# pvjosue/CWFA

Hardware: AMD Instinct MI355X
Metric: volumes/sec inverse-pass @512×512×96 fp32; NLL match vs ref (1/2/4/8 GPU) (higher is better)
Workload: dtype f32 (storage, accumulation, wavelets, couplings); convolution products on the bf16 matrix cores from an exact three-way bf16 split of both fp32 operands, six products per fp32 product: fp32-equivalent; plain-fp32-MFMA figure: fp32_mfma; 1 GPU; 512x512x96 volume, 4-scale CWFA (CAT blocks, 64 ch) + LRNN inverse, z=0, batch 1/GPU, random-init weights (BASELINE.json configs[2]); precision=split, parallelism=replicated x1 (independent volumes per GPU, no collective)

## Files before the change

### cwfa_amd/csrc/conv_split3x3.hip

```cpp
#include "conv_internal.h"

extern int g_cwfa_split_xcd_map;
extern int g_cwfa_split_rows16;

namespace {

constexpr int TR = 8, TC = 32;

template <int KS, int RPW = 4>
struct XG {
    static constexpr int TRW = 2 * RPW, NT = 2 * RPW;
    static constexpr int PAD = KS / 2, XR = TRW + 2 * PAD, XC = TC + 2 * PAD, NTAP = KS * KS;
    static constexpr int EPK = XR * XC;
    static constexpr int KHB = KS == 7 ? 8512 : RPW == 8 ? 9792 : 5440;
    static constexpr int XPB = 2 * KHB;
    static constexpr int XB = 3 * XPB;
    static constexpr bool SPECIAL = KS == 3 && RPW == 4;
    static constexpr int NEK = SPECIAL ? 2 : 3;
    static_assert(EPK * 16 <= KHB && KHB % 256 == 64 && 2 * EPK <= 512 * NEK, "staging entry map");
    static_assert(!SPECIAL || (EPK > 256 && EPK <= 384), "3x3 staging entry map");
    static_assert(KS == 3 || RPW == 4, "7x7: 8-row tiles");
};

template <int MPW, int KS = 3, int RPW = 4, int WM = 4>
struct Geo {
    static constexpr int CT = 16 * MPW * WM;
    static constexpr int WSL = 3 * 4 * CT * 16;
    static constexpr int LDS = 2 * XG<KS, RPW>::XB + 2 * WSL;
    static_assert(LDS <= 160 * 1024, "LDS budget");
};

struct SParams {
    const float* x;
    const void* wp;
    float* y;
    int B, Cin, H, W, Cout, nchunks, nsteps, tiles_x, ntiles, ctiles, xcd_map;
    int nrun;
    int64_t x_bs, y_bs;
    cwfa_conv_opts o;
    cwfa_couple cp;
};

template <int KS, int RPW>
__host__ __device__ constexpr int tap_off(int buf, int tap) { return buf * XG<KS, RPW>::XB + ((tap / KS) * XG<KS, RPW>::XC + tap % KS) * 16; }

enum { EPI_RUNTIME = -1, EPI_COUPLE = -2 };

template <int MPW, bool SIX, bool ADD, int ACT1, int KS = 3, int RPW = 4, int WM = 4, bool F16 = false>
__global__ __launch_bounds__(512, 1) void conv3x3_split_kernel(SParams p) {
    typedef XG<KS, RPW> G;
    constexpr int XC = G::XC, EPK = G::EPK, KHB = G::KHB, XPB = G::XPB, XB = G::XB, NTAP = G::NTAP, PAD = G::PAD;
    constexpr int WN = 8 / WM, RW = G::TRW / WN, NT = 2 * RW;
    constexpr bool SPECIAL = G::SPECIAL;
    static_assert(SPECIAL || ((MPW == 1 || WM != 4) && !ADD), "7x7 / 16-row tiles: the 64-channel and narrow tilings, without a skip add");
    static_assert(WM == 4 || (((KS == 3 && RPW == 8) || KS == 7) && MPW <= 3 && !ADD && ACT1 != EPI_COUPLE),
                  "narrow tilings: 16-row tile (7x7: 8-row), <= 3 m-tiles per wave");
    static_assert(MPW != 3 || WM != 4, "three m-tiles per wave: the 48- / 96-channel tilings only");
    constexpr int CT = 16 * MPW * WM;
    constexpr int WSL = 3 * 4 * CT * 16;
    extern __shared__ __attribute__((aligned(16))) char lds[];
    const int tid = threadIdx.x, lane = tid & 63, c16 = lane & 15, g = lane >> 4;
    const int wave = __builtin_amdgcn_readfirstlane(tid >> 6);
    const int wm = wave % WM, wn = wave / WM;
    const int HW = p.H * p.W;
    const int plane = HW * 4;
    constexpr unsigned OOB = 0x80000000u;
    constexpr int NQ = SIX ? 3 : 1;
    constexpr int OFF_W = 2 * XB;
    const int b = blockIdx.z;
    int sp, ct;
    if (p.xcd_map && (p.ntiles & 7) == 0) {
        const int xcd = blockIdx.x & 7, slot = blockIdx.x >> 3;
        sp = xcd * (p.ntiles >> 3) + slot / p.ctiles;
        ct = slot % p.ctiles;
    } else {
        sp = blockIdx.x / p.ctiles;
        ct = blockIdx.x % p.ctiles;
    }
    const int row0 = (sp / p.tiles_x) * G::TRW, col0 = (sp % p.tiles_x) * TC;

    constexpr int NEK = G::NEK;
    int ekh[NEK], eidx[NEK];
    bool fin[NEK];
    unsigned fo[NEK];
    if constexpr (SPECIAL) {
        ekh[0] = wave >> 2; eidx[0] = tid & 255; fin[0] = true;
        ekh[1] = (wave >> 1) & 1; eidx[1] = 256 + (tid & 127); fin[1] = wave < 4 && eidx[1] < EPK;
    } else {
#pragma unroll
        for (int k = 0; k < NEK; ++k) {
            const int e = tid + 512 * k;
            ekh[k] = e >= EPK;
            eidx[k] = e - ekh[k] * EPK;
            fin[k] = e < 2 * EPK;
        }
    }
    bool fok[NEK];
#pragma unroll
    for (int k = 0; k < NEK; ++k) {
        const int r = eidx[k] / XC, c = eidx[k] % XC;
        const int gr = row0 + r - PAD, gc = col0 + c - PAD;
        fok[k] = fin[k] && gr >= 0 && gr < p.H && gc >= 0 && gc < p.W;
        fo[k] = !fok[k] ? OOB : p.o.in_blocked8 ? (unsigned)((gr * p.W + gc) * 32) : (unsigned)((gr * p.W + gc) * 4);
        if constexpr (!SPECIAL) fo[k] = !fok[k] ? OOB : fo[k] + (unsigned)(ekh[k] * 8) * (unsigned)plane;
    }
    const int xbytes = p.Cin * plane;
    const auto rx = CWFA_RSRC(p.x + (int64_t)b * p.x_bs, xbytes);
    const auto ra = CWFA_RSRC(ADD ? p.o.in_add + (int64_t)b * p.o.in_add_bs : p.x, ADD ? xbytes : 0);
    const bool has_aff = p.o.in_scale != nullptr;
    typedef const float __attribute__((address_space(4))) cfloat;
    cfloat* sc = has_aff ? (cfloat*)(p.o.in_scale + (int64_t)b * p.o.in_affine_bs) : nullptr;
    cfloat* sh = has_aff ? (cfloat*)(p.o.in_shift + (int64_t)b * p.o.in_affine_bs) : nullptr;

    auto load_entry = [&](auto kc, float (&xv)[8], float (&av)[8], int chunk) {
        constexpr int k = decltype(kc)::value;
        const int ch0 = chunk * 16 + (SPECIAL ? ekh[k] * 8 : 0);
        if (KS == 3 && !ADD && p.o.in_blocked8) {
            const f32x4 lo4 = __builtin_bit_cast(f32x4, __builtin_amdgcn_raw_buffer_load_b128(rx, fo[k], ch0 * plane, 0));
            const f32x4 hi4 = __builtin_bit_cast(f32x4, __builtin_amdgcn_raw_buffer_load_b128(rx, fo[k], ch0 * plane + 16, 0));
#pragma unroll
            for (int j = 0; j < 4; ++j) {
                xv[j] = lo4[j];
                xv[4 + j] = hi4[j];
            }
            return;
        }
#pragma unroll
        for (int j = 0; j < 8; ++j) xv[j] = __builtin_bit_cast(float, __builtin_amdgcn_raw_buffer_load_b32(rx, fo[k], (ch0 + j) * plane, 0));
        if constexpr (ADD) {
#pragma unroll
            for (int j = 0; j < 8; ++j) av[j] = __builtin_bit_cast(float, __builtin_amdgcn_raw_buffer_load_b32(ra, fo[k], (ch0 + j) * plane, 0));
        }
    };
    auto store_entry = [&](auto kc, const float (&xv)[8], const float (&av)[8], int chunk, int buf) {
        constexpr int k = decltype(kc)::value;
        if (SPECIAL && k == 1 && !fin[1]) return;
        const int ch0 = chunk * 16 + ekh[k] * 8;
        bf16x8 pc[3];
        float scv[8], shv[8];
        if (has_aff) {
#pragma unroll
            for (int j = 0; j < 8; ++j) {
                const int ch = ch0 + j < p.Cin ? ch0 + j : p.Cin - 1;
                scv[j] = ch0 + j < p.Cin ? sc[ch] : 0.f;
                shv[j] = ch0 + j < p.Cin ? sh[ch] : 0.f;
            }
        }
#pragma unroll
        for (int j = 0; j < 8; ++j) {
            float v = xv[j];
            if (has_aff) v = fok[k] ? v * scv[j] + shv[j] : 0.f;
            if constexpr (ADD) v += av[j];
            __bf16 a1, a2 = (__bf16)0.f, a3 = (__bf16)0.f;
            cwfa_split3<SIX, F16>(v, a1, a2, a3);
            pc[0][j] = a1; pc[1][j] = a2; pc[2][j] = a3;
        }
        char* dst = lds + buf * XB + ekh[k] * KHB + eidx[k] * 16;
        if (SPECIAL || fin[k]) {
#pragma unroll
            for (int q = 0; q < NQ; ++q) *reinterpret_cast<bf16x8*>(dst + q * XPB) = pc[q];
        }
    };

    constexpr int NPC = (SIX ? WSL : WSL / 3) / 1024;
    const int64_t wtile = (int64_t)ct * p.nsteps * WSL;
    const char* wbase = reinterpret_cast<const char*>(p.wp) + wtile;
    const auto rw = CWFA_RSRC(wbase, p.nsteps * WSL);
    auto dma_w = [&](int slice, int slot) {
        cwfa_static_for<(NPC + 7) / 8>([&](auto ic_) {
            constexpr int i = decltype(ic_)::value;
            const int piece = i * 8 + wave;
            if (piece < NPC) {
                char* dst = lds + OFF_W + slot * WSL + piece * 1024;
                __builtin_amdgcn_raw_ptr_buffer_load_lds(rw, (lds_ptr)dst, 16, (unsigned)(lane * 16), slice * WSL + piece * 1024, 0, 0);
            }
        });
    };

    const int alane = OFF_W + (g * CT + wm * MPW * 16 + c16) * 16;
    const int blane = (g & 1) * KHB + (wn * RW * XC + c16) * 16;
    const bool sel = (g >> 1) != 0;

    f32x4 acc[MPW][NT];
#pragma unroll
    for (int mt = 0; mt < MPW; ++mt)
#pragma unroll
        for (int nt = 0; nt < NT; ++nt) acc[mt][nt] = f32x4{0.f, 0.f, 0.f, 0.f};
    constexpr int NB = MPW == 4 ? 3 : 2, MA = MPW == 4 ? 2 : MPW;
    static_assert(NB - 1 < NT, "B look-ahead");
    bf16x8 A[MPW][3], Bq[NB][3];
    float xs[NEK][8], sk[NEK][8];

    auto read_a = [&](int abase, int m0, int m1) {
#pragma unroll
        for (int mt = m0; mt < m1; ++mt)
#pragma unroll
            for (int q = 0; q < NQ; ++q) A[mt][q] = *reinterpret_cast<const bf16x8*>(lds + abase + (q * 4 * CT + mt * 16) * 16);
    };
    auto read_b = [&](int set, int bbase, int nt) {
#pragma unroll
        for (int q = 0; q < NQ; ++q)
            Bq[set][q] = *reinterpret_cast<const bf16x8*>(lds + bbase + q * XPB + ((nt >> 1) * XC + 16 * (nt & 1)) * 16);
    };
    auto mfma6 = [&](f32x4& c, const bf16x8 (&a)[3], const bf16x8 (&bb)[3]) {
        if constexpr (SIX) {
            CWFA_MFMA(a[2], bb[0], c);
            CWFA_MFMA(a[1], bb[1], c);
            CWFA_MFMA(a[0], bb[2], c);
            CWFA_MFMA(a[1], bb[0], c);
            CWFA_MFMA(a[0], bb[1], c);
        }
        CWFA_MFMA_OP(F16, a[0], bb[0], c);
    };

    {
        float x0[NEK][8], s0[NEK][8];
        cwfa_static_for<NEK>([&](auto kc) { load_entry(kc, x0[decltype(kc)::value], s0[decltype(kc)::value], 0); });
        cwfa_static_for<NEK>([&](auto kc) { load_entry(kc, xs[decltype(kc)::value], sk[decltype(kc)::value], 1); });
        dma_w(0, 0);
        cwfa_static_for<NEK>([&](auto kc) { store_entry(kc, x0[decltype(kc)::value], s0[decltype(kc)::value], 0, 0); });
    }
    asm volatile("s_waitcnt vmcnt(0)\n\ts_waitcnt lgkmcnt(0)" ::: "memory");
    __builtin_amdgcn_s_barrier();

    read_b(0, blane + (sel ? tap_off<KS, RPW>(0, 1) : tap_off<KS, RPW>(0, 0)), 0);
    int sl = 0, P = 0, ce = 0;
    for (int step = 0; step < p.nrun; ++step) {
        const int co = ce + 1;
        const int uA = 2 * P, uB = 2 * P + 1;
        const int bufA = uA >= NTAP, tA = uA - NTAP * bufA, bufB = uB >= NTAP, tB = uB - NTAP * bufB;
        const int offA = bufA * XB + ((tA / KS) * XC + tA % KS) * 16, offB = bufB * XB + ((tB / KS) * XC + tB % KS) * 16;
        constexpr int SB = 0, SA = KS == 3 ? 5 : 26, LA = KS == 3 ? 2 : 22, LB = KS == 3 ? 6 : 44;
        static_assert(LB + NEK - 1 < NTAP && LA + NEK - 1 < SA, "staging schedule");
        static_assert(SB < LA && SA <= LB, "staging schedule: one register set per entry (a step's stores come before its loads)");
        {
            const bool odd0 = P == SB, odd1 = P == SB + 1;
            if (odd0 || P == SA) store_entry(cwfa_ic<0>{}, xs[0], sk[0], odd0 ? co : ce + 2, odd0);
            if (odd1 || P == SA + 1) store_entry(cwfa_ic<1>{}, xs[1], sk[1], odd1 ? co : ce + 2, odd1);
            if constexpr (NEK > 2) {
                const bool odd2 = P == SB + 2;
                if (odd2 || P == SA + 2) store_entry(cwfa_ic<NEK - 1>{}, xs[NEK - 1], sk[NEK - 1], odd2 ? co : ce + 2, odd2);
            }
        }
        CWFA_FENCE();
        const int abase = alane + sl * WSL;
        const int bbase = blane + (sel ? offB : offA);
        read_a(abase, 0, MA);
        CWFA_FENCE();
#pragma unroll
        for (int nt = 0; nt < NT; ++nt) {
            if ((MA == MPW || nt > 0) && nt + NB - 1 < NT) read_b((nt + NB - 1) % NB, bbase, nt + NB - 1);
            CWFA_FENCE();
#pragma unroll
            for (int mt = 0; mt < MPW; ++mt) {
                mfma6(acc[mt][nt], A[mt], Bq[nt % NB]);
                CWFA_FENCE();
                if (MA < MPW && nt == 0 && mt == 0) {
                    read_a(abase, MA, MPW);
#pragma unroll
                    for (int n2 = 1; n2 < NB && n2 < NT; ++n2) read_b(n2, bbase, n2);
                    CWFA_FENCE();
                }
            }
            if (nt == 0) {
                if (P == LA || P == LB) load_entry(cwfa_ic<0>{}, xs[0], sk[0], P == LA ? ce + 2 : co + 2);
                if (P == LA + 1 || P == LB + 1) load_entry(cwfa_ic<1>{}, xs[1], sk[1], P == LA + 1 ? ce + 2 : co + 2);
                if constexpr (NEK > 2) {
                    if (P == LA + 2 || P == LB + 2) load_entry(cwfa_ic<NEK - 1>{}, xs[NEK - 1], sk[NEK - 1], P == LA + 2 ? ce + 2 : co + 2);
                }
                CWFA_FENCE();
            }
            if (nt == 1) {
                dma_w(step + 1, sl ^ 1);
                CWFA_FENCE();
            }
        }
        {
            const int nP = P == NTAP - 1 ? 0 : P + 1;
            const int nA = 2 * nP, nB = 2 * nP + 1;
            const int nbufA = nA >= NTAP, ntA = nA - NTAP * nbufA, nbufB = nB >= NTAP, ntB = nB - NTAP * nbufB;
            const int noffA = nbufA * XB + ((ntA / KS) * XC + ntA % KS) * 16, noffB = nbufB * XB + ((ntB / KS) * XC + ntB % KS) * 16;
            read_b(0, blane + (sel ? noffB : noffA), 0);
            CWFA_FENCE();
        }
        asm volatile("s_waitcnt vmcnt(0)" ::: "memory");
        if constexpr (SIX) asm volatile("s_waitcnt lgkmcnt(3)" ::: "memory");
        else asm volatile("s_waitcnt lgkmcnt(1)" ::: "memory");
        __builtin_amdgcn_s_barrier();
        sl ^= 1;
        if (++P == NTAP) {
            P = 0;
            ce += 2;
        }
    }
    asm volatile("s_waitcnt vmcnt(0)" ::: "memory");

    const auto ry = CWFA_RSRC(p.y + (int64_t)b * p.y_bs, p.Cout * plane);
    const auto rr = CWFA_RSRC(p.o.residual ? p.o.residual + (int64_t)b * p.o.res_bs : p.y, p.o.residual ? p.Cout * plane : 0);
    const auto rb = CWFA_RSRC(p.o.bias ? p.o.bias : p.y, p.o.bias ? p.Cout * 4 : 0);
    const bool alpha_pc = p.o.prelu_per_channel != 0;
    const float alpha = (p.o.prelu_alpha && !alpha_pc) ? *p.o.prelu_alpha : 0.f;
    const auto rpa = CWFA_RSRC(alpha_pc ? p.o.prelu_alpha : p.y, alpha_pc ? p.Cout * 4 : 0);
    const int cwave = ct * CT + wm * MPW * 16;
    const unsigned glane = (unsigned)(4 * g) * (unsigned)plane;
    if constexpr (ACT1 == EPI_COUPLE) {
        static_assert(MPW <= 2 && !ADD, "coupling epilogue: narrow tilings only");
        constexpr int NP = MPW == 1 ? 2 : 4;
        const cwfa_couple& cp = p.cp;
        const auto cx = CWFA_RSRC(cp.x + (int64_t)b * cp.x_bs, cp.n * plane);
        const auto cy = CWFA_RSRC(cp.y + (int64_t)b * cp.y_bs, cp.n * plane);
        const unsigned jlane = (unsigned)((MPW == 1 ? 2 : 4) * g) * (unsigned)plane;
        const int jwave = wm * (MPW == 1 ? 8 : 16);
        float bs[NP], bt[NP];
#pragma unroll
        for (int k = 0; k < NP; ++k) {
            const int rs = k, rt = MPW == 1 ? k + 2 : 16 + k;
            bs[k] = __builtin_bit_cast(float, __builtin_amdgcn_raw_buffer_load_b32(rb, (unsigned)(16 * g), (cwave + rs) * 4, 0));
            bt[k] = __builtin_bit_cast(float, __builtin_amdgcn_raw_buffer_load_b32(rb, (unsigned)(16 * g), (cwave + rt) * 4, 0));
        }
        float ssum = 0.f;
#pragma unroll
        for (int nt = 0; nt < NT; ++nt) {
            const int row = row0 + wn * RW + (nt >> 1), col = col0 + 16 * (nt & 1) + c16;
            const bool ok = row < p.H && col < p.W;
            const unsigned po = ok ? (unsigned)((row * p.W + col) * 4) + jlane : OOB;
            float xv[NP];
#pragma unroll
            for (int k = 0; k < NP; ++k) xv[k] = __builtin_bit_cast(float, __builtin_amdgcn_raw_buffer_load_b32(cx, po, (jwave + k) * plane, 0));
#pragma unroll
            for (int k = 0; k < NP; ++k) {
                const float sr = acc[0][nt][k] + bs[k];
                float tr;
                if constexpr (MPW == 1) tr = acc[0][nt][k + 2] + bt[k];
                else tr = acc[MPW - 1][nt][k] + bt[k];
                const float sv = cwfa_soft_clamp(sr * cp.pre_scale, cp.clamp_kind, cp.clamp);
                const float tv = tr * cp.pre_scale;
                const float yv = cp.rev ? (xv[k] - tv) * __expf(-sv) : __expf(sv) * xv[k] + tv;
                __builtin_amdgcn_raw_buffer_store_b32(__builtin_bit_cast(unsigned, yv), cy, po, (jwave + k) * plane, 0);
                ssum += ok ? sv : 0.f;
            }
            CWFA_FENCE();
        }
        if (cp.logdet) {
            const double ws = cwfa_wave_sum((double)ssum);
            double* red = reinterpret_cast<double*>(lds);
            __builtin_amdgcn_s_barrier();
            if (lane == 0) red[wave] = ws;
            __syncthreads();
            if (tid == 0) {
                double tot = 0.0;
#pragma unroll
                for (int w = 0; w < 8; ++w) tot += red[w];
                atomicAdd(&cp.logdet[b], cp.rev ? -tot : tot);
            }
        }
        return;
    }
    const bool outb = p.o.out_blocked8 != 0;
    const bool want_stats = ACT1 != EPI_RUNTIME && p.o.out_stats != nullptr;
    float* red = reinterpret_cast<float*>(lds);
#pragma unroll
    for (int mt = 0; mt < MPW; ++mt) {
        float bias[4];
        float st1[4] = {0.f, 0.f, 0.f, 0.f}, st2[4] = {0.f, 0.f, 0.f, 0.f};
#pragma unroll
        for (int r = 0; r < 4; ++r)
            bias[r] = __builtin_bit_cast(float, __builtin_amdgcn_raw_buffer_load_b32(rb, (unsigned)(16 * g), (cwave + mt * 16 + r) * 4, 0));
        float al[4] = {alpha, alpha, alpha, alpha};
        if (alpha_pc) {
#pragma unroll
            for (int r = 0; r < 4; ++r)
                al[r] = __builtin_bit_cast(float, __builtin_amdgcn_raw_buffer_load_b32(rpa, (unsigned)(16 * g), (cwave + mt * 16 + r) * 4, 0));
        }
        constexpr int RLA = NT < 4 ? NT : 4;
        float rv[ACT1 == EPI_RUNTIME ? NT : 1][4];
        auto load_res = [&](int nt) {
            const int row = row0 + wn * RW + (nt >> 1), col = col0 + 16 * (nt & 1) + c16;
            const unsigned po = (row < p.H && col < p.W) ? (unsigned)((row * p.W + col) * 4) + glane : OOB;
#pragma unroll
            for (int r = 0; r < 4; ++r)
                rv[ACT1 == EPI_RUNTIME ? nt : 0][r] = __builtin_bit_cast(float, __builtin_amdgcn_raw_buffer_load_b32(rr, po, (cwave + mt * 16 + r) * plane, 0));
        };
        if constexpr (ACT1 == EPI_RUNTIME) {
#pragma unroll
            for (int nt = 0; nt < NT; ++nt)
#pragma unroll
                for (int r = 0; r < 4; ++r) rv[nt][r] = 0.f;
            if (p.o.residual) {
#pragma unroll
                for (int nt = 0; nt < RLA; ++nt) load_res(nt);
            }
            CWFA_FENCE();
        }
#pragma unroll
        for (int nt = 0; nt < NT; ++nt) {
            const int row = row0 + wn * RW + (nt >> 1), col = col0 + 16 * (nt & 1) + c16;
            if constexpr (ACT1 == EPI_RUNTIME) {
                if (nt + RLA < NT && p.o.residual) load_res(nt + RLA);
                CWFA_FENCE();
            }
            if constexpr (ACT1 != EPI_RUNTIME) {
                if (outb) {
                    f32x4 o4;
#pragma unroll
                    for (int r = 0; r < 4; ++r) o4[r] = cwfa_act_ct<ACT1>(acc[mt][nt][r] + bias[r], al[r]);
                    const unsigned pb = (row < p.H && col < p.W) ? (unsigned)(((g >> 1) * HW + row * p.W + col) * 32 + (g & 1) * 16) : OOB;
                    cwfa_buffer_store_b128(__builtin_bit_cast(u32x4, o4), ry, pb, (cwave + mt * 16) * plane);
                    continue;
                }
            }
            const unsigned po = (row < p.H && col < p.W) ? (unsigned)((row * p.W + col) * 4) + glane : OOB;
#pragma unroll
            for (int r = 0; r < 4; ++r) {
                const int soff = (cwave + mt * 16 + r) * plane;
                float v = acc[mt][nt][r] + bias[r];
                if constexpr (ACT1 == EPI_RUNTIME) {
                    v = cwfa_act(v, p.o.act, al[r]);
                    v += rv[nt][r];
                    v = cwfa_act(v, p.o.act2, al[r]);
                } else {
                    v = cwfa_act_ct<ACT1>(v, al[r]);
                    if (want_stats) {
                        const float vm = po != OOB ? v : 0.f;
                        st1[r] += vm;
                        st2[r] += vm * vm;
                    }
                }
                __builtin_amdgcn_raw_buffer_store_b32(__builtin_bit_cast(unsigned, v), ry, po, soff, 0);
            }
            CWFA_FENCE();
        }
        if constexpr (ACT1 != EPI_RUNTIME) {
            if (want_stats) {
#pragma unroll
                for (int r = 0; r < 4; ++r) {
                    const float a1 = cwfa_row16_sum(st1[r]), a2 = cwfa_row16_sum(st2[r]);
                    if (c16 == 0) {
                        const int ch = (wm * MPW + mt) * 16 + 4 * g + r;
                        red[(wn * CT + ch) * 2] = a1;
                        red[(wn * CT + ch) * 2 + 1] = a2;
                    }
                }
            }
        }
    }
    if constexpr (ACT1 != EPI_RUNTIME) {
        if (want_stats) {
            asm volatile("s_waitcnt lgkmcnt(0)\n\ts_barrier" ::: "memory");
            const int ch = ct * CT + tid;
            if (tid < CT && ch < p.Cout) {
                double s1 = 0.0, s2 = 0.0;
#pragma unroll
                for (int k = 0; k < WN; ++k) {
                    s1 += (double)red[(k * CT + tid) * 2];
                    s2 += (double)red[(k * CT + tid) * 2 + 1];
                }
                atomicAdd(&p.o.out_stats[2 * ch], s1);
                atomicAdd(&p.o.out_stats[2 * ch + 1], s2);
            }
        }
    }
}

namespace few {
constexpr int XR = TR + 6, XC = TC + 6, EPK = XR * XC;
constexpr int XPB = EPK * 16;
constexpr int NSTEP = 13, CT = 64, MPW = 2, WM = 2, WN = 4, RW = 2, NT = 4;
constexpr int WSL = 3 * 4 * CT * 16;
constexpr int OFF_W = 3 * XPB, LDS = OFF_W + 2 * WSL;
static_assert(2 * 512 >= EPK && 2 * LDS <= 160 * 1024, "few-channel 7x7: staging map / two blocks per CU");
}

template <bool SIX, bool F16>
__global__ __launch_bounds__(512, 2) void conv7x7_few_split_kernel(SParams p) {
    using namespace few;
    extern __shared__ __attribute__((aligned(16))) char lds[];
    const int tid = threadIdx.x, lane = tid & 63, c16 = lane & 15, g = lane >> 4;
    const int wave = __builtin_amdgcn_readfirstlane(tid >> 6);
    const int wm = wave % WM, wn = wave / WM;
    const int plane = p.H * p.W * 4;
    constexpr unsigned OOB = 0x80000000u;
    constexpr int NQ = SIX ? 3 : 1;
    const int b = blockIdx.z;
    int sp;
    if (p.xcd_map && (p.ntiles & 7) == 0) sp = (blockIdx.x & 7) * (p.ntiles >> 3) + (blockIdx.x >> 3);
    else sp = blockIdx.x;
    const int row0 = (sp / p.tiles_x) * TR, col0 = (sp % p.tiles_x) * TC;

    constexpr int NPC = (SIX ? WSL : WSL / 3) / 1024;
    const auto rw = CWFA_RSRC(p.wp, NSTEP * WSL);
    auto dma_w = [&](int slice, int slot) {
        cwfa_static_for<(NPC + 7) / 8>([&](auto ic_) {
            constexpr int i = decltype(ic_)::value;
            const int piece = i * 8 + wave;
            if (piece < NPC) {
                char* dst = lds + OFF_W + slot * WSL + piece * 1024;
                __builtin_amdgcn_raw_ptr_buffer_load_lds(rw, (lds_ptr)dst, 16, (unsigned)(lane * 16), slice * WSL + piece * 1024, 0, 0);
            }
        });
    };

    {
        const auto rx = CWFA_RSRC(p.x + (int64_t)b * p.x_bs, p.Cin * plane);
        float xv[2][8];
#pragma unroll
        for (int k = 0; k < 2; ++k) {
            const int e = tid + 512 * k, r = e / XC, c = e % XC;
            const int gr = row0 + r - 3, gc = col0 + c - 3;
            const bool ok = e < EPK && gr >= 0 && gr < p.H && gc >= 0 && gc < p.W;
            const unsigned fo = ok ? (unsigned)((gr * p.W + gc) * 4) : OOB;
#pragma unroll
            for (int j = 0; j < 8; ++j) xv[k][j] = __builtin_bit_cast(float, __builtin_amdgcn_raw_buffer_load_b32(rx, fo, j * plane, 0));
        }
        dma_w(0, 0);
#pragma unroll
        for (int k = 0; k < 2; ++k) {
            const int e = tid + 512 * k;
            bf16x8 pc[3];
#pragma unroll
            for (int j = 0; j < 8; ++j) {
                __bf16 a1, a2 = (__bf16)0.f, a3 = (__bf16)0.f;
                cwfa_split3<SIX, F16>(xv[k][j], a1, a2, a3);
                pc[0][j] = a1; pc[1][j] = a2; pc[2][j] = a3;
            }
            if (e < EPK) {
#pragma unroll
                for (int q = 0; q < NQ; ++q) *reinterpret_cast<bf16x8*>(lds + q * XPB + e * 16) = pc[q];
            }
        }
    }
    asm volatile("s_waitcnt vmcnt(0)\n\ts_waitcnt lgkmcnt(0)" ::: "memory");
    __builtin_amdgcn_s_barrier();

    const int alane = OFF_W + (g * CT + wm * MPW * 16 + c16) * 16;
    const int blane = (wn * RW * XC + c16) * 16;
    auto bbase_of = [&](int s) {
        const int t = 4 * s + g < 48 ? 4 * s + g : 48;
        return blane + ((t / 7) * XC + t % 7) * 16;
    };

    f32x4 acc[MPW][NT];
#pragma unroll
    for (int mt = 0; mt < MPW; ++mt)
#pragma unroll
        for (int nt = 0; nt < NT; ++nt) acc[mt][nt] = f32x4{0.f, 0.f, 0.f, 0.f};
    bf16x8 A[MPW][3], Bq[2][3];
    auto read_b = [&](int set, int bbase, int nt) {
#pragma unroll
        for (int q = 0; q < NQ; ++q)
            Bq[set][q] = *reinterpret_cast<const bf16x8*>(lds + bbase + q * XPB + ((nt >> 1) * XC + 16 * (nt & 1)) * 16);
    };
    auto mfma6 = [&](f32x4& c, const bf16x8 (&a)[3], const bf16x8 (&bb)[3]) {
        if constexpr (SIX) {
            CWFA_MFMA(a[2], bb[0], c);
            CWFA_MFMA(a[1], bb[1], c);
            CWFA_MFMA(a[0], bb[2], c);
            CWFA_MFMA(a[1], bb[0], c);
            CWFA_MFMA(a[0], bb[1], c);
        }
        CWFA_MFMA_OP(F16, a[0], bb[0], c);
    };

    int bbase = bbase_of(0);
    read_b(0, bbase, 0);
    int sl = 0;
#pragma unroll 1
    for (int step = 0; step < NSTEP; ++step) {
        const int abase = alane + sl * WSL;
#pragma unroll
        for (int mt = 0; mt < MPW; ++mt)
#pragma unroll
            for (int q = 0; q < NQ; ++q) A[mt][q] = *reinterpret_cast<const bf16x8*>(lds + abase + (q * 4 * CT + mt * 16) * 16);
        CWFA_FENCE();
#pragma unroll
        for (int nt = 0; nt < NT; ++nt) {
            if (nt + 1 < NT) read_b((nt + 1) & 1, bbase, nt + 1);
            CWFA_FENCE();
#pragma unroll
            for (int mt = 0; mt < MPW; ++mt) {
                mfma6(acc[mt][nt], A[mt], Bq[nt & 1]);
                CWFA_FENCE();
            }
            if (nt == 0 && step + 1 < NSTEP) {
                dma_w(step + 1, sl ^ 1);
                CWFA_FENCE();
            }
        }
        bbase = bbase_of(step + 1 < NSTEP ? step + 1 : step);
        read_b(0, bbase, 0);
        CWFA_FENCE();
        asm volatile("s_waitcnt vmcnt(0)" ::: "memory");
        if constexpr (SIX) asm volatile("s_waitcnt lgkmcnt(3)" ::: "memory");
        else asm volatile("s_waitcnt lgkmcnt(1)" ::: "memory");
        __builtin_amdgcn_s_barrier();
        sl ^= 1;
    }

    const auto ry = CWFA_RSRC(p.y + (int64_t)b * p.y_bs, p.Cout * plane);
    const auto rb = CWFA_RSRC(p.o.bias ? p.o.bias : p.y, p.o.bias ? p.Cout * 4 : 0);
    const int cwave = wm * MPW * 16;
    const unsigned glane = (unsigned)(4 * g) * (unsigned)plane;
    const bool want_stats = p.o.out_sample_stats != nullptr;
    double ssum = 0.0, ssq = 0.0;
#pragma unroll
    for (int mt = 0; mt < MPW; ++mt) {
        float bias[4];
#pragma unroll
        for (int r = 0; r < 4; ++r)
            bias[r] = __builtin_bit_cast(float, __builtin_amdgcn_raw_buffer_load_b32(rb, (unsigned)(16 * g), (cwave + mt * 16 + r) * 4, 0));
#pragma unroll
        for (int nt = 0; nt < NT; ++nt) {
            const int row = row0 + wn * RW + (nt >> 1), col = col0 + 16 * (nt & 1) + c16;
            const unsigned po = (row < p.H && col < p.W) ? (unsigned)((row * p.W + col) * 4) + glane : OOB;
            float v[4];
#pragma unroll
            for (int r = 0; r < 4; ++r) {
                v[r] = acc[mt][nt][r] + bias[r];
                __builtin_amdgcn_raw_buffer_store_b32(__builtin_bit_cast(unsigned, v[r]), ry, po, (cwave + mt * 16 + r) * plane, 0);
            }
            if (want_stats) {
#pragma unroll
                for (int r = 0; r < 4; ++r) {
                    const double dv = (po != OOB && cwave + mt * 16 + 4 * g + r < p.Cout) ? (double)v[r] : 0.0;
                    ssum += dv;
                    ssq += dv * dv;
                }
            }
            CWFA_FENCE();
        }
    }
    if (want_stats) {
        ssum = cwfa_wave_sum(ssum);
        ssq = cwfa_wave_sum(ssq);
        double* red = reinterpret_cast<double*>(lds);
        if (lane == 0) {
            red[2 * wave] = ssum;
            red[2 * wave + 1] = ssq;
        }
        __syncthreads();
        if (tid == 0) {
            double t1 = 0.0, t2 = 0.0;
#pragma unroll
            for (int w = 0; w < 8; ++w) {
                t1 += red[2 * w];
                t2 += red[2 * w + 1];
            }
            atomicAdd(&p.o.out_sample_stats[2 * b], t1);
            atomicAdd(&p.o.out_sample_stats[2 * b + 1], t2);
        }
    }
}

template <bool F16>
__global__ __launch_bounds__(256) void split7x7_few_pack_kernel(const float* __restrict__ w, uint4* __restrict__ out, int Cout, int Cin) {
    const int i = blockIdx.x * blockDim.x + threadIdx.x;
    if (i >= few::NSTEP * 4 * 64) return;
    const int co = i % 64, g = (i / 64) % 4, s = i / 256, tap = 4 * s + g;
    unsigned short pc[3][8];
#pragma unroll
    for (int j = 0; j < 8; ++j) {
        float v = 0.f;
        if (co < Cout && j < Cin && tap < 49) v = w[((int64_t)co * Cin + j) * 49 + tap];
        __bf16 a1, a2, a3;
        if constexpr (F16) {
            cwfa_split3<false, true>(v, a1, a2, a3);
            a2 = a3 = __builtin_bit_cast(__bf16, (unsigned short)0);
        } else {
            cwfa_split3<true>(v, a1, a2, a3);
        }
        pc[0][j] = __builtin_bit_cast(unsigned short, a1);
        pc[1][j] = __builtin_bit_cast(unsigned short, a2);
        pc[2][j] = __builtin_bit_cast(unsigned short, a3);
    }
#pragma unroll
    for (int q = 0; q < 3; ++q) {
        uint4 v4;
        v4.x = pc[q][0] | ((unsigned)pc[q][1] << 16);
        v4.y = pc[q][2] | ((unsigned)pc[q][3] << 16);
        v4.z = pc[q][4] | ((unsigned)pc[q][5] << 16);
        v4.w = pc[q][6] | ((unsigned)pc[q][7] << 16);
        out[((s * 3 + q) * 4 + g) * 64 + co] = v4;
    }
}

template <int CT, bool F16 = false>
__global__ __launch_bounds__(256) void split3x3_pack_kernel(const float* __restrict__ w, uint4* __restrict__ out, int Cout, int Cin,
                                                            int nchunks, int nsteps, int64_t total, int ntap) {
    const int64_t i = (int64_t)blockIdx.x * blockDim.x + threadIdx.x;
    if (i >= total) return;
    const int col = (int)(i % CT), g = (int)((i / CT) % 4), s = (int)((i / (4 * CT)) % nsteps), ctile = (int)(i / ((int64_t)4 * CT * nsteps));
    const int u = 2 * s + (g >> 1), chunk = u / ntap, tap = u % ntap, co = ctile * CT + col;
    unsigned short pc[3][8];
#pragma unroll
    for (int j = 0; j < 8; ++j) {
        const int ci = chunk * 16 + (g & 1) * 8 + j;
        float v = 0.f;
        if (co < Cout && ci < Cin && chunk < nchunks) v = w[((int64_t)co * Cin + ci) * ntap + tap];
        __bf16 a1, a2, a3;
        if constexpr (F16) {
            cwfa_split3<false, true>(v, a1, a2, a3);
            a2 = a3 = __builtin_bit_cast(__bf16, (unsigned short)0);
        } else {
            cwfa_split3<true>(v, a1, a2, a3);
        }
        pc[0][j] = __builtin_bit_cast(unsigned short, a1);
        pc[1][j] = __builtin_bit_cast(unsigned short, a2);
        pc[2][j] = __builtin_bit_cast(unsigned short, a3);
    }
#pragma unroll
    for (int q = 0; q < 3; ++q) {
        uint4 v4;
        v4.x = pc[q][0] | ((unsigned)pc[q][1] << 16);
        v4.y = pc[q][2] | ((unsigned)pc[q][3] << 16);
        v4.z = pc[q][4] | ((unsigned)pc[q][5] << 16);
        v4.w = pc[q][6] | ((unsigned)pc[q][7] << 16);
        out[(((int64_t)ctile * nsteps + s) * 3 + q) * 4 * CT + g * CT + col] = v4;
    }
}

inline int mpw_of(int Cout) { return Cout > 128 ? 4 : Cout > 96 ? 2 : Cout > 64 ? 3 : Cout > 48 ? 1 : Cout > 32 ? 3 : Cout > 16 ? 2 : 1; }
inline int wm_of(int Cout) { return Cout > 96 ? 4 : Cout > 64 ? 2 : Cout > 48 ? 4 : 1; }
inline int ct_of(int Cout) { return 16 * mpw_of(Cout) * wm_of(Cout); }
inline int nsteps_of(int Cin, int ntap = 9) { return ntap * (((Cin + 15) / 16 + 1) / 2); }

template <int MPW, bool ADD, int ACT1, int KS = 3, int RPW = 4, int WM = 4>
int launch(const SParams& p, hipStream_t stream) {
    typedef Geo<MPW, KS, RPW, WM> G;
    constexpr int TRW = XG<KS, RPW>::TRW;
    const int tiles_y = (p.H + TRW - 1) / TRW, ctiles = (p.Cout + G::CT - 1) / G::CT;
    SParams q = p;
    q.ntiles = p.tiles_x * tiles_y;
    q.ctiles = ctiles;
    q.xcd_map = g_cwfa_split_xcd_map;
    if ((int64_t)q.ntiles * ctiles >= (1ll << 31)) {
        cwfa_set_error("cwfa_conv3x3_split_f32: grid too large");
        return CWFA_E_SHAPE;
    }
    if ((ACT1 == EPI_RUNTIME || ACT1 == EPI_COUPLE) && (p.o.out_stats || p.o.out_blocked8)) {
        cwfa_set_error("cwfa_conv3x3_split_f32: out_stats / out_blocked8 reached a run-time epilogue");
        return CWFA_E_INVAL;
    }
    return cwfa_with_operand([&](auto six, auto f16) -> int {
        constexpr auto kern = &conv3x3_split_kernel<MPW, six, ADD, ACT1, KS, RPW, WM, f16>;
        const int rc = cwfa_max_lds<kern>(G::LDS, "cwfa_conv3x3_split_f32");
        if (rc) return rc;
        hipLaunchKernelGGL(kern, dim3((unsigned)(q.ntiles * ctiles), 1, p.B), dim3(512), G::LDS, stream, q);
        CWFA_LAUNCH_CHECK("cwfa_conv3x3_split_f32");
        return CWFA_OK;
    });
}

template <int MPW>
int launch_epi(const SParams& p, hipStream_t st) {
    const bool plain = !p.o.residual && p.o.act2 == CWFA_ACT_NONE;
    if (p.o.in_add) {
        if (plain && p.o.act == CWFA_ACT_PRELU) return launch<MPW, true, CWFA_ACT_PRELU>(p, st);
        return launch<MPW, true, EPI_RUNTIME>(p, st);
    }
    if (plain && p.o.act == CWFA_ACT_PRELU) return launch<MPW, false, CWFA_ACT_PRELU>(p, st);
    if (plain && p.o.act == CWFA_ACT_NONE) return launch<MPW, false, CWFA_ACT_NONE>(p, st);
    return launch<MPW, false, EPI_RUNTIME>(p, st);
}

void pack_bank(const float* w, void* packed, int Cout, int Cin, int ct, int ntap, hipStream_t st) {
    const int nchunks = (Cin + 15) / 16, nsteps = nsteps_of(Cin, ntap);
    const int64_t total = (int64_t)((Cout + ct - 1) / ct) * nsteps * 4 * ct;
    cwfa_with_operand([&](auto, auto f16) -> int {
        auto go = [&](auto CT) {
            hipLaunchKernelGGL((split3x3_pack_kernel<decltype(CT)::value, f16>), dim3((unsigned)((total + 255) / 256)), dim3(256), 0, st, w,
                               reinterpret_cast<uint4*>(packed), Cout, Cin, nchunks, nsteps, total, ntap);
        };
        if (ct == 16) go(cwfa_ic<16>{});
        else if (ct == 32) go(cwfa_ic<32>{});
        else if (ct == 48) go(cwfa_ic<48>{});
        else if (ct == 96) go(cwfa_ic<96>{});
        else if (ct == 128) go(cwfa_ic<128>{});
        else if (ct == 256) go(cwfa_ic<256>{});
        else go(cwfa_ic<64>{});
        return CWFA_OK;
    });
}

}

static int couple_row_source(int n, int r) {
    int j, which;
    if (n <= 32) {
        const int wm = r >> 4, g = (r >> 2) & 3, q = r & 3;
        j = 8 * wm + 2 * g + (q & 1);
        which = q >> 1;
    } else {
        const int wm = r >> 5;
        which = (r >> 4) & 1;
        j = 16 * wm + (r & 15);
    }
    return j < n ? which * n + j : -1;
}

extern "C" int cwfa_couple_rows(int n, int* rows) {
    if (n <= 0 || n > 64) return -1;
    const int total = n <= 32 ? 64 : 128;
    if (rows)
        for (int r = 0; r < total; ++r) rows[r] = couple_row_source(n, r);
    return total;
}

extern "C" int cwfa_conv3x3_split_couple_f32(const float* x, const void* w_packed, const float* bias_rows, int B, int Cin, int H, int W,
                                             int64_t x_bs, const cwfa_couple* cp, void* stream) {
    CWFA_REQUIRE(B >= 0 && Cin > 0 && H >= 0 && W >= 0, CWFA_E_INVAL, "cwfa_conv3x3_split_couple_f32: bad size");
    CWFA_REQUIRE(cp, CWFA_E_INVAL, "cwfa_conv3x3_split_couple_f32: null coupling descriptor");
    CWFA_REQUIRE(cp->n > 0 && cp->n <= 64, CWFA_E_SHAPE, "cwfa_conv3x3_split_couple_f32: 1 <= n <= 64 (got %d)", cp->n);
    if (B == 0 || H == 0 || W == 0) return CWFA_OK;
    CWFA_REQUIRE(x && w_packed && cp->x && cp->y, CWFA_E_INVAL, "cwfa_conv3x3_split_couple_f32: null pointer");
    CWFA_REQUIRE(cwfa_aligned16(w_packed), CWFA_E_ALIGN, "cwfa_conv3x3_split_couple_f32: packed weights must be 16-byte aligned");
    CWFA_REQUIRE(cp->clamp_kind >= CWFA_CLAMP_NONE && cp->clamp_kind <= CWFA_CLAMP_SIGMOID, CWFA_E_INVAL,
                 "cwfa_conv3x3_split_couple_f32: bad clamp kind %d", cp->clamp_kind);
    SParams p{};
    p.x = x; p.wp = w_packed; p.y = cp->y;
    p.B = B; p.Cin = Cin; p.H = H; p.W = W; p.x_bs = x_bs; p.y_bs = cp->y_bs;
    p.Cout = cwfa_couple_rows(cp->n, nullptr);
    p.o.bias = bias_rows;
    p.o.in_blocked8 = cp->in_blocked8;
    CWFA_REQUIRE(!cp->in_blocked8 || (Cin % 8 == 0 && cwfa_aligned16(x) && (x_bs & 3) == 0), CWFA_E_ALIGN,
                 "cwfa_conv3x3_split_couple_f32: blocked input needs Cin %% 8 == 0 and 16-byte alignment");
    p.cp = *cp;
    p.nchunks = (Cin + 15) / 16;
    p.nsteps = nsteps_of(Cin);
    p.nrun = p.nsteps - ((p.nchunks & 1) ? 4 : 0);
    p.tiles_x = (W + TC - 1) / TC;
    CWFA_REQUIRE((int64_t)(Cin + 64) * H * W * 4 < (1ll << 31) && (int64_t)(cp->n + 64) * H * W * 4 < (1ll << 31), CWFA_E_SHAPE,
                 "cwfa_conv3x3_split_couple_f32: one sample's input / active half must stay below 2 GiB");
    CWFA_REQUIRE((int64_t)p.tiles_x * ((H + TR - 1) / TR) < (1ll << 31) && B <= 65535, CWFA_E_SHAPE,
                 "cwfa_conv3x3_split_couple_f32: grid too large");
    hipStream_t st = (hipStream_t)stream;
    if (p.Cout == 64) {
        if (g_cwfa_split_rows16 && H > 8)
            return launch<1, false, EPI_COUPLE, 3, 8>(p, st);
        return launch<1, false, EPI_COUPLE>(p, st);
    }
    return launch<2, false, EPI_COUPLE>(p, st);
}

extern "C" int64_t cwfa_conv3x3_split_packed_bytes(int Cout, int Cin) {
    if (Cout <= 0 || Cin <= 0) return -1;
    const int ct = ct_of(Cout);
    return (int64_t)((Cout + ct - 1) / ct) * nsteps_of(Cin) * 3 * 4 * ct * 16;
}

extern "C" int cwfa_conv3x3_split_pack_f32(const float* w, void* packed, int Cout, int Cin, void* stream) {
    CWFA_REQUIRE(w && packed, CWFA_E_INVAL, "cwfa_conv3x3_split_pack_f32: null pointer");
    CWFA_REQUIRE(Cout > 0 && Cin > 0, CWFA_E_SHAPE, "cwfa_conv3x3_split_pack_f32: bad shape");
    CWFA_REQUIRE(cwfa_aligned16(packed), CWFA_E_ALIGN, "cwfa_conv3x3_split_pack_f32: packed image must be 16-byte aligned");
    pack_bank(w, packed, Cout, Cin, ct_of(Cout), 9, (hipStream_t)stream);
    CWFA_LAUNCH_CHECK("cwfa_conv3x3_split_pack_f32");
    return CWFA_OK;
}

extern "C" int cwfa_conv3x3_split_f32(const float* x, const void* w_packed, float* y, int B, int Cin, int H, int W, int Cout,
                                      int64_t x_bs, int64_t y_bs, const cwfa_conv_opts* opts, void* stream) {
    CWFA_REQUIRE(B >= 0 && Cin > 0 && Cout > 0 && H >= 0 && W >= 0, CWFA_E_INVAL, "cwfa_conv3x3_split_f32: bad size");
    if (B == 0 || H == 0 || W == 0) return CWFA_OK;
    CWFA_REQUIRE(x && w_packed && y, CWFA_E_INVAL, "cwfa_conv3x3_split_f32: null pointer");
    CWFA_REQUIRE(cwfa_aligned16(w_packed), CWFA_E_ALIGN, "cwfa_conv3x3_split_f32: packed weights must be 16-byte aligned");
    SParams p{};
    p.x = x; p.wp = w_packed; p.y = y;
    p.B = B; p.Cin = Cin; p.H = H; p.W = W; p.Cout = Cout; p.x_bs = x_bs; p.y_bs = y_bs;
    if (opts) p.o = *opts;
    CWFA_REQUIRE(!p.o.upshuffle2 && !p.o.in_cat, CWFA_E_SHAPE, "cwfa_conv3x3_split_f32: upshuffle2 / in_cat are 1x1 features");
    CWFA_REQUIRE(!p.o.out_sample_stats, CWFA_E_INVAL, "cwfa_conv3x3_split_f32: out_sample_stats is a feature of the few-channel cwfa_conv7x7_split_f32");
    CWFA_REQUIRE(!p.o.in_blocked8 || (Cin % 8 == 0 && cwfa_aligned16(x) && (x_bs & 3) == 0 && !p.o.in_add), CWFA_E_ALIGN,
                 "cwfa_conv3x3_split_f32: blocked input needs Cin %% 8 == 0, 16-byte alignment and no added tensor");
    CWFA_REQUIRE(!p.o.out_blocked8 || (Cout % 8 == 0 && cwfa_aligned16(y) && (y_bs & 3) == 0 && !p.o.residual && p.o.act2 == CWFA_ACT_NONE &&
                                       (p.o.act == CWFA_ACT_NONE || p.o.act == CWFA_ACT_PRELU)),
                 CWFA_E_ALIGN, "cwfa_conv3x3_split_f32: blocked output needs Cout %% 8 == 0, 16-byte alignment and a bias / PReLU epilogue");
    CWFA_REQUIRE(!(p.o.in_scale && !p.o.in_shift), CWFA_E_INVAL, "cwfa_conv3x3_split_f32: in_scale without in_shift");
    CWFA_REQUIRE(!p.o.out_stats || (!p.o.out_blocked8 && !p.o.residual && p.o.act2 == CWFA_ACT_NONE &&
                                    (p.o.act == CWFA_ACT_NONE || p.o.act == CWFA_ACT_PRELU)),
                 CWFA_E_INVAL, "cwfa_conv3x3_split_f32: out_stats needs an NCHW output and a bias / PReLU epilogue");
    CWFA_REQUIRE(!((p.o.out_stats || p.o.out_blocked8) && p.o.in_add && p.o.act == CWFA_ACT_NONE), CWFA_E_INVAL,
                 "cwfa_conv3x3_split_f32: out_stats / out_blocked8 with in_add need a PReLU epilogue");
    CWFA_REQUIRE(p.o.act >= 0 && p.o.act <= CWFA_ACT_RELU && p.o.act2 >= 0 && p.o.act2 <= CWFA_ACT_RELU, CWFA_E_INVAL,
                 "cwfa_conv3x3_split_f32: bad activation");
    CWFA_REQUIRE(!((p.o.act == CWFA_ACT_PRELU || p.o.act2 == CWFA_ACT_PRELU) && !p.o.prelu_alpha), CWFA_E_INVAL,
                 "cwfa_conv3x3_split_f32: PReLU without prelu_alpha");
    p.nchunks = (Cin + 15) / 16;
    p.nsteps = nsteps_of(Cin);
    p.nrun = p.nsteps - ((p.nchunks & 1) ? 4 : 0);
    p.tiles_x = (W + TC - 1) / TC;
    const int mpw = mpw_of(Cout);
    CWFA_REQUIRE((int64_t)(Cin + 64) * H * W * 4 < (1ll << 31) && (int64_t)(Cout + 64 * mpw) * H * W * 4 < (1ll << 31) &&
                     (int64_t)(p.nsteps + 2) * 3 * 4 * 64 * mpw * 16 < (1ll << 31), CWFA_E_SHAPE,
                 "cwfa_conv3x3_split_f32: one sample's input / output / one cout tile's weights must stay below 2 GiB");
    CWFA_REQUIRE((int64_t)p.tiles_x * ((H + TR - 1) / TR) < (1ll << 31) && B <= 65535, CWFA_E_SHAPE, "cwfa_conv3x3_split_f32: grid too large");
    hipStream_t st = (hipStream_t)stream;
    const int wm = wm_of(Cout);
    if (wm != 4) {
        CWFA_REQUIRE(!p.o.in_scale && !p.o.in_add && !p.o.out_blocked8, CWFA_E_INVAL,
                     "cwfa_conv3x3_split_f32: banks with <= 48 or 65 .. 96 outputs take no load-side prologue and write NCHW");
        const bool plain = !p.o.residual && p.o.act2 == CWFA_ACT_NONE;
        const int epi = plain && p.o.act == CWFA_ACT_NONE ? 0 : plain && p.o.act == CWFA_ACT_PRELU ? 1 : 2;
#define CWFA_NARROW(M, W_)                                                                                                                   \
    do {                                                                                                                                     \
        if (epi == 0) return launch<M, false, CWFA_ACT_NONE, 3, 8, W_>(p, st);                                                               \
        if (epi == 1) return launch<M, false, CWFA_ACT_PRELU, 3, 8, W_>(p, st);                                                              \
        return launch<M, false, EPI_RUNTIME, 3, 8, W_>(p, st);                                                                               \
    } while (0)
        if (mpw == 3 && wm == 2) CWFA_NARROW(3, 2);
        if (mpw == 3) CWFA_NARROW(3, 1);
        if (mpw == 2) CWFA_NARROW(2, 1);
        CWFA_NARROW(1, 1);
#undef CWFA_NARROW
    }
    if (mpw == 4) return launch_epi<4>(p, st);
    if (mpw == 2) return launch_epi<2>(p, st);
    if (g_cwfa_split_rows16 && H > 8 && !p.o.in_scale && !p.o.in_add && !p.o.residual && p.o.act == CWFA_ACT_NONE && p.o.act2 == CWFA_ACT_NONE)
        return launch<2, false, CWFA_ACT_NONE, 3, 8, 2>(p, st);
    if (g_cwfa_split_rows16 && H > 8 && !p.o.in_scale && !p.o.in_add && !p.o.out_stats && !p.o.out_blocked8)
        return launch<2, false, EPI_RUNTIME, 3, 8, 2>(p, st);
    return launch_epi<1>(p, st);
}

extern "C" int64_t cwfa_conv7x7_split_packed_bytes(int Cout, int Cin) {
    if (Cout <= 0 || Cout > 64 || Cin <= 0) return -1;
    if (Cin <= 8) return (int64_t)few::NSTEP * few::WSL;
    return (int64_t)nsteps_of(Cin, 49) * 3 * 4 * 64 * 16;
}

extern "C" int cwfa_conv7x7_split_pack_f32(const float* w, void* packed, int Cout, int Cin, void* stream) {
    CWFA_REQUIRE(w && packed, CWFA_E_INVAL, "cwfa_conv7x7_split_pack_f32: null pointer");
    CWFA_REQUIRE(Cout > 0 && Cout <= 64 && Cin > 0, CWFA_E_SHAPE, "cwfa_conv7x7_split_pack_f32: 1 <= Cout <= 64");
    CWFA_REQUIRE(cwfa_aligned16(packed), CWFA_E_ALIGN, "cwfa_conv7x7_split_pack_f32: packed image must be 16-byte aligned");
    if (Cin <= 8) {
        cwfa_with_operand([&](auto, auto f16) -> int {
            hipLaunchKernelGGL((split7x7_few_pack_kernel<f16>), dim3((few::NSTEP * 4 * 64 + 255) / 256), dim3(256), 0, (hipStream_t)stream, w,
                               reinterpret_cast<uint4*>(packed), Cout, Cin);
            return CWFA_OK;
        });
    } else {
        pack_bank(w, packed, Cout, Cin, 64, 49, (hipStream_t)stream);
    }
    CWFA_LAUNCH_CHECK("cwfa_conv7x7_split_pack_f32");
    return CWFA_OK;
}

extern "C" int cwfa_conv7x7_split_f32(const float* x, const void* w_packed, float* y, int B, int Cin, int H, int W, int Cout,
                                      int64_t x_bs, int64_t y_bs, const cwfa_conv_opts* opts, void* stream) {
    CWFA_REQUIRE(B >= 0 && Cin > 0 && Cout > 0 && Cout <= 64 && H >= 0 && W >= 0, CWFA_E_INVAL, "cwfa_conv7x7_split_f32: bad size (Cout <= 64)");
    if (B == 0 || H == 0 || W == 0) return CWFA_OK;
    CWFA_REQUIRE(x && w_packed && y, CWFA_E_INVAL, "cwfa_conv7x7_split_f32: null pointer");
    CWFA_REQUIRE(cwfa_aligned16(w_packed), CWFA_E_ALIGN, "cwfa_conv7x7_split_f32: packed weights must be 16-byte aligned");
    SParams p{};
    p.x = x; p.wp = w_packed; p.y = y;
    p.B = B; p.Cin = Cin; p.H = H; p.W = W; p.Cout = Cout; p.x_bs = x_bs; p.y_bs = y_bs;
    if (opts) p.o = *opts;
    CWFA_REQUIRE(!p.o.upshuffle2 && !p.o.in_cat && !p.o.in_scale && !p.o.in_add && !p.o.in_blocked8 && !p.o.out_blocked8 && !p.o.residual && !p.o.out_stats &&
                     p.o.act == CWFA_ACT_NONE && p.o.act2 == CWFA_ACT_NONE,
                 CWFA_E_INVAL, "cwfa_conv7x7_split_f32: bias-only epilogue, no load-side prologue, NCHW maps");
    CWFA_REQUIRE(!p.o.out_sample_stats || Cin <= 8, CWFA_E_INVAL, "cwfa_conv7x7_split_f32: out_sample_stats is written by the few-channel form (Cin <= 8) only");
    p.nchunks = (Cin + 15) / 16;
    p.nsteps = nsteps_of(Cin, 49);
    p.nrun = p.nchunks == 1 ? 25 : p.nsteps;
    p.tiles_x = (W + TC - 1) / TC;
    CWFA_REQUIRE((int64_t)(Cin + 64) * H * W * 4 < (1ll << 31) && (int64_t)(Cout + 64) * H * W * 4 < (1ll << 31), CWFA_E_SHAPE,
                 "cwfa_conv7x7_split_f32: one sample's input / output must stay below 2 GiB");
    CWFA_REQUIRE((int64_t)p.tiles_x * ((H + TR - 1) / TR) < (1ll << 31) && B <= 65535, CWFA_E_SHAPE, "cwfa_conv7x7_split_f32: grid too large");
    hipStream_t st = (hipStream_t)stream;
    if (Cin <= 8) {
        p.ntiles = p.tiles_x * ((H + TR - 1) / TR);
        p.ctiles = 1;
        p.xcd_map = g_cwfa_split_xcd_map;
        return cwfa_with_operand([&](auto six, auto f16) -> int {
            constexpr auto kern = &conv7x7_few_split_kernel<six, f16>;
            const int rc = cwfa_max_lds<kern>(few::LDS, "cwfa_conv7x7_split_f32");
            if (rc) return rc;
            hipLaunchKernelGGL(kern, dim3((unsigned)p.ntiles, 1, B), dim3(512), few::LDS, st, p);
            CWFA_LAUNCH_CHECK("cwfa_conv7x7_split_f32");
            return CWFA_OK;
        });
    }
    return launch<2, false, CWFA_ACT_NONE, 7, 4, 2>(p, st);
}
```

Baseline: 57.32 volumes/s.

## Move per-step barrier to mid-step and prefetch weights two steps ahead

For non-ADD variants of the split-bf16 3x3 conv kernel, the per-step barrier moves from the end of the step to the middle of the n-tile loop. Weight DMA is issued two steps ahead into the current slot, and the next step's A fragments and first B fragments are read during the last n-tile. Staging stores now run after the mid-step barrier. The aim is to hide barrier and LDS latency behind MFMA work, at the cost of a more intricate schedule, with static_asserts guarding its hazards and an extra barrier before the stats reduction.

```diff
diff --git a/cwfa_amd/csrc/conv_split3x3.hip b/cwfa_amd/csrc/conv_split3x3.hip
--- a/cwfa_amd/csrc/conv_split3x3.hip
+++ b/cwfa_amd/csrc/conv_split3x3.hip
@@ -188,6 +188,7 @@
         for (int nt = 0; nt < NT; ++nt) acc[mt][nt] = f32x4{0.f, 0.f, 0.f, 0.f};
     constexpr int NB = MPW == 4 ? 3 : 2, MA = MPW == 4 ? 2 : MPW;
     static_assert(NB - 1 < NT, "B look-ahead");
+    constexpr bool MIDSTEP = !ADD;
     bf16x8 A[MPW][3], Bq[NB][3];
     float xs[NEK][8], sk[NEK][8];
 
@@ -218,11 +219,13 @@
         cwfa_static_for<NEK>([&](auto kc) { load_entry(kc, x0[decltype(kc)::value], s0[decltype(kc)::value], 0); });
         cwfa_static_for<NEK>([&](auto kc) { load_entry(kc, xs[decltype(kc)::value], sk[decltype(kc)::value], 1); });
         dma_w(0, 0);
+        if constexpr (MIDSTEP) dma_w(1, 1);
         cwfa_static_for<NEK>([&](auto kc) { store_entry(kc, x0[decltype(kc)::value], s0[decltype(kc)::value], 0, 0); });
     }
     asm volatile("s_waitcnt vmcnt(0)\n\ts_waitcnt lgkmcnt(0)" ::: "memory");
     __builtin_amdgcn_s_barrier();
 
+    if constexpr (MIDSTEP) read_a(alane, 0, MA);
     read_b(0, blane + (sel ? tap_off<KS, RPW>(0, 1) : tap_off<KS, RPW>(0, 0)), 0);
     int sl = 0, P = 0, ce = 0;
     for (int step = 0; step < p.nrun; ++step) {
@@ -231,9 +234,15 @@
         const int bufA = uA >= NTAP, tA = uA - NTAP * bufA, bufB = uB >= NTAP, tB = uB - NTAP * bufB;
         const int offA = bufA * XB + ((tA / KS) * XC + tA % KS) * 16, offB = bufB * XB + ((tB / KS) * XC + tB % KS) * 16;
         constexpr int SB = 0, SA = KS == 3 ? 5 : 26, LA = KS == 3 ? 2 : 22, LB = KS == 3 ? 6 : 44;
+        constexpr int MID = NT / 2;
+        constexpr int FO = (NTAP - 1) / 2;
         static_assert(LB + NEK - 1 < NTAP && LA + NEK - 1 < SA, "staging schedule");
         static_assert(SB < LA && SA <= LB, "staging schedule: one register set per entry (a step's stores come before its loads)");
-        {
+        static_assert(!MIDSTEP || SB + NEK - 1 <= FO - 2, "staging schedule: the odd buffer is complete one barrier before the end of step FO - 1");
+        static_assert(!MIDSTEP || (SA >= FO + 1 && SA + NEK - 1 <= NTAP - 2), "staging schedule: the even buffer is written behind mid(FO + 1) ... mid(NTAP - 2)");
+        static_assert(MID >= 1 && MID + NB - 2 < NT, "mid-step barrier: the B look-ahead it leaves outstanding lies inside the step");
+        constexpr int LOAD_NT = MIDSTEP ? MID : 0, DMA_NT = !MIDSTEP ? 1 : NT >= 8 ? MID + 1 : MID;
+        auto staging_stores = [&]() {
             const bool odd0 = P == SB, odd1 = P == SB + 1;
             if (odd0 || P == SA) store_entry(cwfa_ic<0>{}, xs[0], sk[0], odd0 ? co : ce + 2, odd0);
             if (odd1 || P == SA + 1) store_entry(cwfa_ic<1>{}, xs[1], sk[1], odd1 ? co : ce + 2, odd1);
@@ -241,15 +250,28 @@
                 const bool odd2 = P == SB + 2;
                 if (odd2 || P == SA + 2) store_entry(cwfa_ic<NEK - 1>{}, xs[NEK - 1], sk[NEK - 1], odd2 ? co : ce + 2, odd2);
             }
-        }
-        CWFA_FENCE();
-        const int abase = alane + sl * WSL;
+            CWFA_FENCE();
+        };
+        const int abase = alane + sl * WSL, anext = alane + (sl ^ 1) * WSL;
         const int bbase = blane + (sel ? offB : offA);
-        read_a(abase, 0, MA);
-        CWFA_FENCE();
+        auto read_b_next = [&]() {
+            const int nP = P == NTAP - 1 ? 0 : P + 1;
+            const int nA = 2 * nP, nB = 2 * nP + 1;
+            const int nbufA = nA >= NTAP, ntA = nA - NTAP * nbufA, nbufB = nB >= NTAP, ntB = nB - NTAP * nbufB;
+            const int noffA = nbufA * XB + ((ntA / KS) * XC + ntA % KS) * 16, noffB = nbufB * XB + ((ntB / KS) * XC + ntB % KS) * 16;
+            read_b(0, blane + (sel ? noffB : noffA), 0);
+            CWFA_FENCE();
+        };
+        static_assert((NT - 1) % NB != 0 && NT >= 2, "the last n-tile is not multiplied from B set 0 (the next step's first fragments land there)");
+        if constexpr (!MIDSTEP) {
+            staging_stores();
+            read_a(abase, 0, MA);
+            CWFA_FENCE();
+        }
 #pragma unroll
         for (int nt = 0; nt < NT; ++nt) {
             if ((MA == MPW || nt > 0) && nt + NB - 1 < NT) read_b((nt + NB - 1) % NB, bbase, nt + NB - 1);
+            if (MIDSTEP && nt == NT - 1) read_b_next();
             CWFA_FENCE();
 #pragma unroll
             for (int mt = 0; mt < MPW; ++mt) {
@@ -261,8 +283,18 @@
                     for (int n2 = 1; n2 < NB && n2 < NT; ++n2) read_b(n2, bbase, n2);
                     CWFA_FENCE();
                 }
-            }
-            if (nt == 0) {
+                if (MIDSTEP && nt == NT - 1 && mt < MA) {
+                    read_a(anext, mt, mt + 1);
+                    CWFA_FENCE();
+                }
+            }
+            if (MIDSTEP && nt == MID - 1) {
+                asm volatile("s_waitcnt vmcnt(0)" ::: "memory");
+                asm volatile("s_waitcnt lgkmcnt(%0)" ::"n"((NB - 1) * NQ) : "memory");
+                __builtin_amdgcn_s_barrier();
+                staging_stores();
+            }
+            if (nt == LOAD_NT) {
                 if (P == LA || P == LB) load_entry(cwfa_ic<0>{}, xs[0], sk[0], P == LA ? ce + 2 : co + 2);
                 if (P == LA + 1 || P == LB + 1) load_entry(cwfa_ic<1>{}, xs[1], sk[1], P == LA + 1 ? ce + 2 : co + 2);
                 if constexpr (NEK > 2) {
@@ -270,23 +302,18 @@
                 }
                 CWFA_FENCE();
             }
-            if (nt == 1) {
-                dma_w(step + 1, sl ^ 1);
+            if (nt == DMA_NT) {
+                if constexpr (MIDSTEP) dma_w(step + 2, sl);
+                else dma_w(step + 1, sl ^ 1);
                 CWFA_FENCE();
             }
         }
-        {
-            const int nP = P == NTAP - 1 ? 0 : P + 1;
-            const int nA = 2 * nP, nB = 2 * nP + 1;
-            const int nbufA = nA >= NTAP, ntA = nA - NTAP * nbufA, nbufB = nB >= NTAP, ntB = nB - NTAP * nbufB;
-            const int noffA = nbufA * XB + ((ntA / KS) * XC + ntA % KS) * 16, noffB = nbufB * XB + ((ntB / KS) * XC + ntB % KS) * 16;
-            read_b(0, blane + (sel ? noffB : noffA), 0);
-            CWFA_FENCE();
-        }
-        asm volatile("s_waitcnt vmcnt(0)" ::: "memory");
-        if constexpr (SIX) asm volatile("s_waitcnt lgkmcnt(3)" ::: "memory");
-        else asm volatile("s_waitcnt lgkmcnt(1)" ::: "memory");
-        __builtin_amdgcn_s_barrier();
+        if constexpr (!MIDSTEP) read_b_next();
+        if constexpr (!MIDSTEP) {
+            asm volatile("s_waitcnt vmcnt(0)" ::: "memory");
+            asm volatile("s_waitcnt lgkmcnt(%0)" ::"n"(NQ) : "memory");
+            __builtin_amdgcn_s_barrier();
+        }
         sl ^= 1;
         if (++P == NTAP) {
             P = 0;
@@ -432,6 +459,7 @@
         }
         if constexpr (ACT1 != EPI_RUNTIME) {
             if (want_stats) {
+                if (MIDSTEP && mt == 0) asm volatile("s_waitcnt lgkmcnt(0)\n\ts_barrier" ::: "memory");
 #pragma unroll
                 for (int r = 0; r < 4; ++r) {
                     const float a1 = cwfa_row16_sum(st1[r]), a2 = cwfa_row16_sum(st2[r]);
```

Result: faster. 58.08 volumes/s, median of 6 (+1.3%).
